# ALLabMTL/marl-demandresponse

Hardware: AMD Instinct MI355X
Metric: house-steps/s (env.step throughput) at 1M houses; % HBM roofline (higher is better)
Workload: dtype f64; 1 GPU; 1,048,576 houses per GPU, random actions, fused FSM+thermal+reward step, every tick's reward row written (BASELINE metric at 1M houses; configs[1]'s controller); houses_per_gpu=1048576, houses_total=1048576, signal=sinusoidals, penalty=individual_L2, action_mode=random, chunk_ticks=128, window_ticks=32, parallelism=1 GPU

## Files before the change

### include/mdr.h

```cpp
#ifndef MDR_H_
#define MDR_H_

#include <stdint.h>

#ifdef __cplusplus
extern "C" {
#endif

#define MDR_ABI_VERSION 5
#define MDR_MAX_CAP 64

enum {
  MDR_OK = 0,
  MDR_EARG = -1,
  MDR_EHIP = -2,
  MDR_ERCCL = -3,
  MDR_ENOMEM = -4,
  MDR_ESTATE = -5,
};

enum { MDR_PEN_INDIVIDUAL_L2 = 0, MDR_PEN_COMMON_L2 = 1, MDR_PEN_COMMON_MAX = 2, MDR_PEN_MIXTURE = 3 };

enum {
  MDR_ACT_BUFFER = 0,
// ... 52 lines not shown
const char* mdr_build_id(void);
int mdr_abi_sizes(int64_t* out, int n);
const char* mdr_last_error(void);
int mdr_graph_info(mdr_ctx* ctx, int64_t* out, int n);
int mdr_graph_memset_probe(mdr_ctx* ctx, int64_t* out, int n, void* stream);
int mdr_create(mdr_ctx** out, const mdr_config* cfg);
int mdr_destroy(mdr_ctx* ctx);
int mdr_bind(mdr_ctx* ctx, const mdr_soa* soa);

int mdr_params_changed(mdr_ctx* ctx);

enum { MDR_OPT_STEP_TPW = 1, MDR_OPT_FASTDIV = 2, MDR_OPT_WINDOW_PIPELINE = 3, MDR_OPT_SHARDED_OVERLAP = 4,
       MDR_OPT_GREEDY_SORT = 5, MDR_OPT_FORCE_HALO = 6, MDR_OPT_WINDOW_THERMAL = 7,
       MDR_OPT_HALO_OVERLAP = 9, MDR_OPT_ACTOR_GENERIC = 10, MDR_OPT_HALO_IN_COUNTS = 12,
       MDR_OPT_GQ_BAND = 13, MDR_OPT_ACTOR_FP32_FORM = 14, MDR_OPT_GQ_FUSED = 15, MDR_OPT_GQ_ADAPTIVE = 16,
       MDR_OPT_ACTOR_GRID = 17 };
enum { MDR_FP32_F16_SPLIT = 0, MDR_FP32_BF16_SPLIT3 = 1 };
enum { MDR_THERMAL_EXACT = 0, MDR_THERMAL_AFFINE = 1 };
int mdr_set_option(mdr_ctx* ctx, int option, int64_t value);

size_t mdr_window_onb_bytes(int64_t n_local, int waves);
int mdr_window_geometry_check(int64_t n_local, size_t onb_bytes, size_t wah_bytes);
size_t mdr_window_pen_bytes(int64_t n_local);
int mdr_window_pen_check(int64_t n_local, size_t pen_bytes);
size_t mdr_window_stats_bytes(int64_t n_local);
int mdr_window_stats_check(int64_t n_local, size_t bytes);

typedef struct mdr_pop_spec {
  double target_temp, std_target;
  double thermo_lo, thermo_hi;
  double ca, cm, hm;
  double init_air, init_mass;
  int32_t n_draw;
  uint8_t draw_idx[MDR_MAX_CAP];
} mdr_pop_spec;
int mdr_populate(mdr_ctx* ctx, const mdr_pop_spec* spec, void* stream);

// ... 207 lines not shown
```

### marl-demandresponse_amd/csrc/mdr_capi.hip

```cpp
#include <hip/hip_ext.h>
#include <hip/hip_runtime.h>
#include <hipcub/hipcub.hpp>
#include <rccl/rccl.h>

#include <cmath>
#include <cstdio>
#include <cstdlib>
#include <cstring>
#include <map>
#include <string>
#include <tuple>
#include <vector>

#include "mdr_actor.h"
#include "mdr_devbuf.h"
#include "mdr_interp.h"
#include "mdr_obs_dev.h"
#include "mdr_kernels.h"

using namespace mdr;

namespace {

thread_local std::string g_err;
// ... 102 lines not shown
  bool actor_generic = false;
  int actor_grid = 0;
  bool actor_fp32_bf16 = false;
  bool halo_overlap = true;
  bool halo_in_counts = true;
  Dev<unsigned long long> d_c5;
  int thermal = MDR_THERMAL_AFFINE;
  int win = kWindowMax;
  Dev<unsigned long long> d_wslab;
  int wslab_len = 0;
  bool wslab_dirty = true;
  Dev<uint64_t> d_onb;
  Dev<uint32_t> d_wah;
  Dev<uint64_t> d_onb2;
  Dev<uint32_t> d_wah2;
  bool coef_dirty = true;
  Dev<int> d_flags;
  Dev<unsigned> d_tickets;
  Dev<TickArgs> d_ticks;
  std::map<GraphKey, std::pair<hipGraphExec_t, int>> graphs;
  int64_t g_cap = 0;
  Dev<double> g_key, g_key2, g_ps, g_incl;
  Dev<int> g_idx, g_idx2;
  Dev<uint8_t> g_ls;
  Dev<unsigned char> g_tmp;
  Dev<int64_t> g_kpos, g_extra;
  Dev<double> g_part;
  Dev<unsigned> g_hist;
  Dev<unsigned char> g_sel_rec;
  GqSel* g_sel = nullptr;
// ... 30 lines not shown
    void* user = nullptr;
  } host;
  int world = 1, rank = 0;
  hipStream_t comm_stream = nullptr;
  hipStream_t cap_stream = nullptr;
  hipEvent_t ev_k1[kSlabs] = {}, ev_ar[kSlabs] = {}, ev_pc = nullptr;
  hipEvent_t ev[16] = {};
  std::vector<hipEvent_t>* step_events = nullptr;
  struct {
    bool on = false;
    int n = 0, mode = 0;
    uint64_t tick0 = 0;
    const uint8_t* action = nullptr;
    int64_t act_stride = 0;
    bool sharded = false;
  } begun;
  Dev<unsigned char> d_actor;
  Dev<float> d_actor_raw;
  std::vector<int> actor_key;
  mdr_actor_spec actor{};
  mdr_actor_net net{};
  bool actor_ready = false;
  int actor_head = MDR_HEAD_SOFTMAX;
  Dev<float> d_eps;
  Dev<float> d_chain;
  int n_cu = 0;
  Dev<double> d_obs_sc;
  Dev<uint8_t> d_act;
  Dev<float> d_halo;
  Dev<double> d_stats;
// ... 342 lines not shown
    for (int i = 0; i < cfg->n_cap; ++i) ok = ok && fabs(tab[i]) < 1099511627776.0;
    k.fast_tick_ok = ok ? 1 : 0;
  }
  c->slab_len = kCountShards * cfg->n_cap;
  if (c->d_slab.reserve((size_t)kSlabs * c->slab_len))
    return cleanup(fail(MDR_ENOMEM, "count slabs"));
  if (hipMemset(c->d_slab, 0, kSlabs * c->slab_len * sizeof(unsigned long long)) != hipSuccess)
    return cleanup(fail(MDR_EHIP, "count slabs memset"));
  c->tpw = default_tpw(cfg->n_local);
  if (cfg->n_cap <= kWindowCap) {
    c->wslab_len = kWindowMax * kCountShards * cfg->n_cap + kWindowMax * cfg->n_cap + kWindowMax * kWindowRec;
    const size_t tiles64 = whole_blocks(win_tiles(cfg->n_local) + 1, kCountWaves) * kWinHpt + 1;
    if (c->d_wslab.reserve((size_t)3 * c->wslab_len) || c->d_onb.reserve(tiles64 * kWindowMax) ||
        c->d_wah.reserve((size_t)cfg->n_local + 1))
      return cleanup(fail(MDR_ENOMEM, "window count slabs"));
  } else {
    c->win = 0;
  }
  c->pen_blocks = (int)blocks(cfg->n_local, 512);
  if (c->d_pen_partial.reserve((size_t)2 * c->pen_blocks) || c->d_partial2.reserve(2))
    return cleanup(fail(MDR_ENOMEM, "penalty partials"));
  if (cfg->penalty_mode != MDR_PEN_INDIVIDUAL_L2 && c->d_wslab) {
    if (c->d_wpen.reserve(mdr_window_pen_bytes(cfg->n_local) / sizeof(double)) || c->d_wres.reserve(3 * kWindowMax))
      return cleanup(fail(MDR_ENOMEM, "window penalty partials"));
  }
  for (auto& e : c->ev)
    if (hipEventCreate(&e) != hipSuccess) return cleanup(fail(MDR_EHIP, "event"));
  for (int i = 0; i < kSlabs; ++i)
    if (hipEventCreateWithFlags(&c->ev_k1[i], hipEventDisableTiming) != hipSuccess ||
        hipEventCreateWithFlags(&c->ev_ar[i], hipEventDisableTiming) != hipSuccess)
// ... 66 lines not shown
    case MDR_OPT_ACTOR_GRID:
      if (value < 0) return fail(MDR_EARG, "mdr_set_option: ACTOR_GRID must be >= 0");
      c->actor_grid = (int)std::min<int64_t>(value, (int64_t)c->n_cu);
      break;
    case MDR_OPT_ACTOR_FP32_FORM:
      if (value != MDR_FP32_F16_SPLIT && value != MDR_FP32_BF16_SPLIT3)
        return fail(MDR_EARG, "mdr_set_option: ACTOR_FP32_FORM must be MDR_FP32_F16_SPLIT or MDR_FP32_BF16_SPLIT3");
      c->actor_fp32_bf16 = value == MDR_FP32_BF16_SPLIT3;
      c->actor_key.clear();
      break;
    case MDR_OPT_WINDOW_THERMAL:
      if (value != MDR_THERMAL_EXACT && value != MDR_THERMAL_AFFINE)
        return fail(MDR_EARG, "mdr_set_option: WINDOW_THERMAL must be MDR_THERMAL_EXACT or _AFFINE");
      c->thermal = (int)value;
      break;
    default: return fail(MDR_EARG, "mdr_set_option: unknown option");
  }
  HIP_TRY(hipDeviceSynchronize());
  destroy_graphs(c);
  return MDR_OK;
}

int mdr_bind(mdr_ctx* c, const mdr_soa* s) {
  drop_begun(c);
  if (!c || !s) return fail(MDR_EARG, "mdr_bind: null argument");
  if (!s->t_air || !s->t_mass || !s->hvac || !s->ua || !s->ca || !s->cm || !s->hm || !s->target ||
      !s->cap_idx)
    return fail(MDR_EARG, "mdr_bind: null array");
  KParams& k = c->kp;
  k.t_air = s->t_air;
// ... 171 lines not shown
}

static bool window_ok(const mdr_ctx* c, int mode) {
  return window_geom_ok(c) && (win_common(c) ? c->d_wpen != nullptr : true) &&
         (mode == MDR_ACT_RANDOM || mode == MDR_ACT_ALWAYS_ON || mode == MDR_ACT_BUFFER);
}

static bool closed_ok(const mdr_ctx* c, int mode, bool stats = false) {
  return window_geom_ok(c) && (win_common(c) ? !stats && c->d_wpen && c->d_wres : true) &&
         (mode == MDR_ACT_BANGBANG || mode == MDR_ACT_DEADBAND_BANGBANG);
}

static int wslab_clean(mdr_ctx* c, hipStream_t st) {
  if (!c->wslab_dirty || !c->d_wslab) return MDR_OK;
  HIP_TRY(hipMemsetAsync(c->d_wslab, 0, 3 * sizeof(unsigned long long) * c->wslab_len, st));
  c->wslab_dirty = false;
  return MDR_OK;
}

static unsigned win_grid(const mdr_ctx* c, int waves = 4) {
  return (unsigned)(whole_blocks(win_tiles(c->kp.n), waves) / waves);
}

extern "C" size_t mdr_window_onb_bytes(int64_t n_local, int waves) {
  if (n_local < 0 || waves < 1) return 0;
  return whole_blocks(win_tiles(n_local), waves) * kWinHpt * kWindowMax * sizeof(uint64_t);
}

extern "C" int mdr_window_geometry_check(int64_t n_local, size_t onb_bytes, size_t wah_bytes) {
  if (n_local < 1) return fail(MDR_EARG, "window launch: no houses");
  const size_t need = std::max(mdr_window_onb_bytes(n_local, kCountWaves), mdr_window_onb_bytes(n_local, 4));
  if (onb_bytes < need)
    return fail(MDR_EARG, "window launch: ON-mask rows of " + std::to_string(onb_bytes) + " B, the launch geometry touches " +
                              std::to_string(need) + " B");
  if (wah_bytes < (size_t)n_local * sizeof(uint32_t))
    return fail(MDR_EARG, "window launch: end-word buffer shorter than the shard");
  return MDR_OK;
}

extern "C" size_t mdr_window_pen_bytes(int64_t n_local) {
  if (n_local < 0) return 0;
  return whole_blocks(win_tiles(n_local), 4) * kWindowMax * 2 * sizeof(double);
}

extern "C" int mdr_window_pen_check(int64_t n_local, size_t pen_bytes) {
  if (n_local < 1) return fail(MDR_EARG, "window launch: no houses for the penalty partial rows");
  const size_t need = mdr_window_pen_bytes(n_local);
  if (pen_bytes < need)
    return fail(MDR_EARG, "window launch: penalty partial rows of " + std::to_string(pen_bytes) +
                              " B, the launch geometry writes " + std::to_string(need) + " B");
  return MDR_OK;
// ... 182 lines not shown
  for (int j = 0; j < K; ++j) {
    const mdr_tick& h = host_ticks[j];
    dv.od_k[j] = h.t_od_prev + 273.0;
    dv.solar[j] = h.solar;
    dv.s_prev[j] = h.s_prev;
    if (fabs(h.t_od_prev) < 1048576.0 && fabs(h.solar) < 1099511627776.0) dv.ok |= 1u << j;
  }
  dv.tick0 = host_ticks[0].tick;
  if (nw == 1) dv.p_out = a.p_out;
  if (first == kBegunAllreduced) dv.red = win_red_ptr(c, s.slot(0));
  if (int rc = s.step(0, nw > 1 ? s.plan.size(1) : 0, c->d_onb, c->d_wah, s.slot(1), &dv)) return rc;
  if (int rc = s.finish(0)) return rc;
  if (a.n > K)
    if (int rc = stage_recs(host_ticks + K, a.n - K, c->d_ticks + K, st)) return rc;
  if (int rc = s.staged_windows(1, false)) return rc;
  c->wslab_dirty = false;
  return MDR_OK;
}

static int window_pipeline(mdr_ctx* c, const RolloutArgs& a, hipStream_t st) {
  if (int rc = win_common_unsharded(c, true)) return rc;
  const WinSeq s{c, a, st, WinPlan(a.n, c->win)};
  const int nw = s.plan.count();
  hipStream_t cs = c->comm_stream;
  uint64_t* onbs[2] = {c->d_onb, c->d_onb2};
  uint32_t* wahs[2] = {c->d_wah, c->d_wah2};
  c->wslab_dirty = true;
  HIP_TRY(hipEventRecord(c->ev_pc, st));
  HIP_TRY(hipStreamWaitEvent(cs, c->ev_pc, 0));
  for (int w = 0; w < nw; ++w) {
// ... 267 lines not shown

int mdr_rollout_stats(mdr_ctx* c, int n, const mdr_tick* ticks, const uint8_t* action, int64_t act_stride,
                      int mode, double* reward, int64_t rew_stride, double* p_out, double* stats, int row0,
                      int use_graph, void* stream) {
  const RolloutArgs a{n, action, act_stride, mode, reward, rew_stride, p_out};
  const char* const who = stats ? "mdr_rollout_stats" : "mdr_rollout";
  if (int rc = rollout_preamble(c, who, ticks && a.reward, a, 0)) return rc;
  if (stats) {
    if (row0 < 0) return fail(MDR_EARG, std::string(who) + ": row0 < 0");
    if (int rc = rollout_stats_path(c, a.mode, who); rc < 0) return rc;
  }
  if (common_sharded(c))
    return fail(MDR_EARG, std::string(who) + ": common penalty modes on a sharded context need the per-step API");
  hipStream_t st = S(stream);
  double* const srow = stats ? stats + (size_t)row0 * kTickRow : nullptr;
  const bool counted = begun_matches(c, a, ticks, false);
  if (c->begun.on && !counted) c->wslab_dirty = true;
  c->begun.on = false;
  int rc = refresh_if_dirty(c, st);
  if (rc) return rc;
  if (counted || (!use_graph && window_ok(c, a.mode) && consecutive(ticks, a.n))) {
    rc = ensure_ticks(c, a.n);
    if (!rc) rc = wslab_clean(c, st);
    if (!rc) rc = window_launches_direct(c, a, ticks, counted ? kBegun : kCountNow, st);
    c->counts_ready = false;
    return rc;
  }
  rc = stage_ticks(c, a.n, ticks, st);
  if (!rc) rc = wslab_clean(c, st);
  if (!rc && stats) rc = rollout_stats_scratch(c, a.mode, !a.p_out);
  if (rc) return rc;
  if (!use_graph) {
    rc = rollout_launches(c, a, st, srow);
    c->counts_ready = false;
    return rc;
  }
  const GraphKey key{a, stats, stats ? row0 : 0};
  auto it = c->graphs.find(key);
  if (it == c->graphs.end()) {
// ... 22 lines not shown

int mdr_rollout_begin(mdr_ctx* c, int n, uint64_t tick0, const uint8_t* action, int64_t act_stride, int mode,
                      void* stream) {
  const RolloutArgs a{n, action, act_stride, mode, nullptr, 0, nullptr};
  if (int rc = rollout_preamble(c, "mdr_rollout_begin", true, a, 0)) return rc;
  if (c->begun.on) c->wslab_dirty = true;
  c->begun.on = false;
  if (!window_ok(c, mode)) return MDR_OK;
  const bool sharded = has_comm(c);
  if (sharded && n > c->win) return MDR_OK;
  if (common_sharded(c)) return MDR_OK;
  hipStream_t st = S(stream);
  int rc = refresh_if_dirty(c, st);
  if (!rc) rc = wslab_clean(c, st);
  if (rc) return rc;
  const int k0 = WinPlan(n, c->win).size(0);
  c->wslab_dirty = true;
  rc = launch_count(c, mode, action, act_stride, nullptr, tick0, k0, c->d_wslab, c->d_onb, c->d_wah, nullptr, st,
                    true);
  if (rc) return rc;
  if (sharded) {
    if (int rc2 = comm_allreduce(c, win_red_ptr(c, c->d_wslab), (size_t)k0 * c->kp.n_cap, 0, st)) return rc2;
  }
  c->wslab_dirty = false;
  c->begun = {true, n, mode, tick0, action, act_stride, sharded};
  return MDR_OK;
}

int mdr_time_step_kernels(mdr_ctx* c, int n, const mdr_tick* ticks, const uint8_t* action, int64_t act_stride,
                          int mode, double* reward, int64_t rew_stride, void* stream, float* ms, int* launches) {
// ... 1816 lines not shown
```

### marl-demandresponse_amd/csrc/mdr_kernels.h

```cpp
#pragma once
#include <hip/hip_runtime.h>
#include <stdint.h>

#include "../../include/mdr.h"

namespace mdr {

constexpr int kCountShards = 64;
constexpr int kWinShards = 16;
constexpr int kCountWaves = 16;
constexpr int kTicketGroups = 64;
constexpr int kTicketWords = 32 * (kTicketGroups + 1);
constexpr int kSlabs = 4;
constexpr int kObsBlock = 128;
constexpr int kActBangBang = 16;
constexpr int kActDeadband = 17;

struct KParams {
  int64_t n, goff, n_global;
  int dt, L, n_cap, penalty_mode;
  double deadband, alpha_temp, alpha_sig, norm_temp, norm_sig;
  double alpha_ind_l2, alpha_common_l2, alpha_common_max;
  uint64_t seed;
  double* t_air;
// ... 123 lines not shown
                              unsigned long long* slot, W... wstat);
__global__ void k_closed_reward(KParams p, const double* rec, int j0, double* reward, int64_t rew_stride);
__global__ void k_closed_reward_common(KParams p, const double* res, const double* rec, int j0, double* reward,
                                       int64_t rew_stride);
__global__ void k_win_shard_sum(KParams p, unsigned long long* slot);
__global__ void k_closed_reward_sharded(KParams p, const unsigned long long* red, const TickArgs* tkp, int j0, int nt,
                                        double* reward, int64_t rew_stride, double* p_out);
__global__ void k_reward_finalize_dev(KParams p, const TickArgs* tkp, const unsigned long long* counts,
                                      const double* partial2, double* reward);
__global__ void k_win_reduce(KParams p, unsigned long long* slot, int nt, const TickArgs* tkp, double* p_out);
__global__ void k_win_records(KParams p, unsigned long long* slot, int nt, const TickArgs* tkp, double* p_out);
template <int ACT, int HPT>
__global__ void k_count_window(KParams p, const uint8_t* action, int64_t act_stride, const TickArgs* tkp,
                               uint64_t tick0, int nt, unsigned long long* slot, uint64_t* onb, uint32_t* wah,
                               const uint32_t* w_in, unsigned* ticket);
__global__ void k_probe_stream(KParams p, double* reward);
__global__ void k_refresh(KParams p, int* params_bad);
__global__ void k_div_check(const double* a, const double* b, int64_t n, unsigned long long* mismatches);
__global__ void k_pen_reduce(const double* pen_partial, int nblk, double* partial2);
__global__ void k_reward_finalize(KParams p, TickArgs tk, const unsigned long long* counts,
                                  const double* partial2, double* reward);
__global__ void k_reward_state(KParams p, const TickArgs* tkp, const unsigned long long* counts,
                               double* reward, double* p_out);
__global__ void k_populate(KParams p, PopArgs a);
constexpr int kStats = 12;
constexpr int kStatsBlocks = 512;
__global__ void k_cluster_stats(KParams p, const double* reward, double* partial);
__global__ void k_cluster_stats_final(const double* partial, int nblk, double* out);
constexpr int kTickRow = 16;
constexpr int kTickBlock = 256;
// ... 101 lines not shown
```

### marl-demandresponse_amd/csrc/mdr_kernels.hip

```cpp
#include "mdr_kernels.h"

#include <tuple>
#include <type_traits>

#include "mdr_device.h"
#include "mdr_obs_dev.h"

namespace mdr {


__device__ __forceinline__ void count_on(bool on, int cls, int n_cap, unsigned* hist,
                                         unsigned long long* slab) {
  const int lane = threadIdx.x & 63;
  for (int k = 0; k < n_cap; ++k) {
    const unsigned long long m = __ballot(on && cls == k);
    if (lane == 0 && m) atomicAdd(&hist[k], (unsigned)__popcll(m));
  }
  __syncthreads();
  if ((int)threadIdx.x < n_cap) {
    const unsigned v = hist[threadIdx.x];
    if (v) atomicAdd(&slab[(blockIdx.x % kCountShards) * n_cap + threadIdx.x],
                     (unsigned long long)v);
  }
}
// ... 933 lines not shown
    if (__hip_atomic_fetch_add(&tickets[32 * g], 1u, __ATOMIC_RELAXED, __HIP_MEMORY_SCOPE_AGENT) == gsize - 1u) {
      __hip_atomic_store(&tickets[32 * g], 0u, __ATOMIC_RELAXED, __HIP_MEMORY_SCOPE_AGENT);
      unsigned* top = &tickets[32 * kTicketGroups];
      if (__hip_atomic_fetch_add(top, 1u, __ATOMIC_RELAXED, __HIP_MEMORY_SCOPE_AGENT) == G - 1u) {
        __hip_atomic_store(top, 0u, __ATOMIC_RELAXED, __HIP_MEMORY_SCOPE_AGENT);
        last = 1u;
      }
    }
    s_last = last;
  }
  __syncthreads();
  return s_last != 0u;
}

template <int NTH>
__device__ void win_reduce_last(const KParams& p, unsigned long long* __restrict__ slot, int nt,
                                unsigned* __restrict__ ticket) {
  static_assert(kWinShards == 16, "one 16-lane group per entry");
  constexpr int EPT = kWinMax * kWinCap * kWinShards / NTH;
  constexpr int EPK = NTH / 16;
  __shared__ unsigned long long s_red[kWinMax * kWinCap];
  if (!grid_last_block(ticket)) return;
  __builtin_amdgcn_fence(__ATOMIC_ACQUIRE, "wavefront");
  const int ncap = p.n_cap, E = nt * ncap, sh = threadIdx.x & 15;
  unsigned long long v[EPT];
#pragma unroll
  for (int k = 0; k < EPT; ++k) {
    const int e = (int)(threadIdx.x >> 4) + EPK * k;
    v[k] = 0ull;
    if (e < E) {
      const int j = e / ncap, c = e - j * ncap;
      v[k] = __hip_atomic_load(&slot[((size_t)j * kCountShards + sh) * ncap + c], __ATOMIC_RELAXED,
                               __HIP_MEMORY_SCOPE_AGENT);
    }
  }
#pragma unroll
  for (int k = 0; k < EPT; ++k) {
    const int e = (int)(threadIdx.x >> 4) + EPK * k;
// ... 3 lines not shown
                         __HIP_MEMORY_SCOPE_AGENT);
    }
    unsigned long long x = v[k];
#pragma unroll
    for (int off = 8; off > 0; off >>= 1) x += __shfl_xor(x, off);
    if (sh == 0 && e < E) s_red[e] = x;
  }
  __syncthreads();
  for (int e = threadIdx.x; e < E; e += blockDim.x) win_red(slot, ncap)[e] = s_red[e];
  if ((int)threadIdx.x < nt) {
    double p_on[kWinCap];
#pragma unroll
    for (int k = 0; k < kWinCap; ++k) p_on[k] = p.p_on[k < ncap ? k : 0];
    win_rec(slot, ncap)[threadIdx.x * kWinRec] = win_power(p, s_red + threadIdx.x * ncap, p_on);
  }
}

template <int HPT>
struct WinTile {
  uint32_t tile, i0;
  uint32_t idx[HPT];
  bool v[HPT];
  uint64_t g0;
  int sh;
  __device__ __forceinline__ WinTile(const KParams& p) {
    const uint32_t n = (uint32_t)p.n;
    const uint32_t wv = (uint32_t)__builtin_amdgcn_readfirstlane((int)(threadIdx.x >> 6));
    tile = blockIdx.x * (blockDim.x >> 6) + wv;
    i0 = tile * (64u * HPT) + (uint32_t)(threadIdx.x & 63);
#pragma unroll
// ... 137 lines not shown
#pragma unroll
  for (int h = 0; h < HPT; ++h) {
    w[h] = w_in ? w_in[t.idx[h]] : p.hvac[t.idx[h]];
    cls[h] = p.cap_idx[t.idx[h]];
  }
  uint64_t cm[HPT][kWinCap];
  win_classes<HPT>(t, cls, cm);
  win_run<ACT, HPT>(p, w, cm, t, tkp, tick0, nt, action, act_stride, s_cnt[wv],
                    onb + (size_t)t.tile * HPT * kWinMax);
#pragma unroll
  for (int h = 0; h < HPT; ++h)
    if (t.v[h]) wah[t.i0 + 64u * h] = w[h];
  __syncthreads();
  win_flush<kCountWaves>(p, nt, s_cnt, slot);
  if (ticket) win_reduce_last<64 * kCountWaves>(p, slot, nt, ticket);
}

struct AffWin {
  double tt, tm, tq, to, qt;
  double mt, mm, mq, mo, qm;
};

__device__ __forceinline__ AffWin aff_window(double ua, double ca, double cm, double hm, double dt, double qc,
                                             bool fast) {
  const RcCoef k = fast ? rc_coeffs_t<true>(ua, ca, cm, hm, dt) : rc_coeffs_t<false>(ua, ca, cm, hm, dt);
  const double iD = 1.0 / (k.r2 - k.r1), iCa = 1.0 / ca, iUa = 1.0 / ua;
  const double a_t = (k.r2 + (ua + hm) * iCa) * iD;
  const double a_m = -(hm * iCa) * iD;
  const double a_q = -(iCa + k.r2 * iUa) * iD;
  const double a_o = -(ua * iCa + k.r2) * iD;
// ... 228 lines not shown

  if (la_K > 0) {
    uint64_t cmk[HPT][kWinCap];
    win_classes<HPT>(t, cls, cmk);
    win_run<ACT, HPT>(p, w_end, cmk, t, KA ? nullptr : tkp + K, KA ? dv.tick0 + (uint64_t)K : 0, la_K,
                      ACT == MDR_ACT_BUFFER ? action + (int64_t)K * act_stride : nullptr, act_stride, s_cnt[wv],
                      onb_w);
#pragma unroll
    for (int h = 0; h < HPT; ++h)
      if (t.v[h]) wah[t.i0 + 64u * h] = w_end[h];
    __syncthreads();
    win_flush(p, la_K, s_cnt, next_slot);
  }
}

constexpr int kClosedSums = 8;
constexpr int kClosedTr = 68;
struct ClosedLds {
  double tr[4][kClosedSums + 1][kClosedTr];
  double ws[4][kWinMax][kStats];
};
__device__ __forceinline__ ClosedLds& closed_lds() {
  __shared__ ClosedLds s;
  return s;
}
template <bool STATS> struct ClosedAcc {};
template <> struct ClosedAcc<true> {
  double a[kClosedSums], mx;
  uint32_t n_lock, n_on;
};
// ... 261 lines not shown
                                                                      unsigned long long*, WinDrv, WinPen);
#define MDR_INST_WIN_F(A, SI, KA_, FO) MDR_INST_WIN_C(A, SI, KA_, FO, false)
#define MDR_INST_WIN(A)                                                                                         \
  MDR_INST_WIN_C(A, false, false, MDR_THERMAL_EXACT, true) MDR_INST_WIN_C(A, false, true, MDR_THERMAL_EXACT, true)   \
  MDR_INST_WIN_C(A, false, false, MDR_THERMAL_AFFINE, true) MDR_INST_WIN_C(A, false, true, MDR_THERMAL_AFFINE, true) \
  MDR_INST_WIN_F(A, true, false, MDR_THERMAL_EXACT) MDR_INST_WIN_F(A, false, false, MDR_THERMAL_EXACT)          \
  MDR_INST_WIN_F(A, true, true, MDR_THERMAL_EXACT) MDR_INST_WIN_F(A, false, true, MDR_THERMAL_EXACT)            \
  MDR_INST_WIN_F(A, true, false, MDR_THERMAL_AFFINE) MDR_INST_WIN_F(A, false, false, MDR_THERMAL_AFFINE)        \
  MDR_INST_WIN_F(A, true, true, MDR_THERMAL_AFFINE) MDR_INST_WIN_F(A, false, true, MDR_THERMAL_AFFINE)          \
  template __global__ void k_count_window<A, kWinHpt>(KParams, const uint8_t*, int64_t, const TickArgs*, uint64_t, \
                                                      int, unsigned long long*, uint64_t*, uint32_t*, const uint32_t*, \
                                                      unsigned*);
MDR_INST_WIN(MDR_ACT_RANDOM)
MDR_INST_WIN(MDR_ACT_ALWAYS_ON)
MDR_INST_WIN(MDR_ACT_BUFFER)

#define MDR_INST_PIPE(T, A, LA, G)                                                                    \
  template __global__ void k_step_pipe<T, A, LA, G>(KParams, const uint8_t*, TickArgs, const TickArgs*, \
                                                    const unsigned long long*, double*, double*,         \
                                                    unsigned long long*, unsigned long long*, GqOut, GqfBufs, int);
MDR_INST_PIPE(1, MDR_ACT_RANDOM, MDR_ACT_RANDOM, 0)
MDR_INST_PIPE(2, MDR_ACT_RANDOM, MDR_ACT_RANDOM, 0)
MDR_INST_PIPE(4, MDR_ACT_RANDOM, MDR_ACT_RANDOM, 0)
MDR_INST_PIPE(8, MDR_ACT_RANDOM, MDR_ACT_RANDOM, 0)
MDR_INST_PIPE(2, MDR_ACT_BUFFER, 0, 0)
MDR_INST_PIPE(4, MDR_ACT_BUFFER, 0, 0)
MDR_INST_PIPE(2, MDR_ACT_BUFFER, 0, 1)
MDR_INST_PIPE(4, MDR_ACT_BUFFER, 0, 1)
MDR_INST_PIPE(2, MDR_ACT_BUFFER, 0, 2)
MDR_INST_PIPE(4, MDR_ACT_BUFFER, 0, 2)
// ... 2310 lines not shown
```

### marl-demandresponse_amd/mdr_amd/_lib.py

```python
from __future__ import annotations

import ctypes as C
import os
import threading

HERE = os.path.dirname(os.path.abspath(__file__))
LIB_PATH = os.environ.get("MDR_LIB", os.path.join(HERE, "libmdr_hip.so"))

ABI_VERSION = 5
MAX_CAP = 64

ACT_BUFFER, ACT_RANDOM, ACT_ALWAYS_ON, ACT_BANGBANG, ACT_DEADBAND_BANGBANG = 0, 1, 2, 16, 17
CTRL_NONE, CTRL_BANGBANG, CTRL_DEADBAND_BANGBANG, CTRL_GREEDY_KEYS = 0, 1, 2, 3
COMM_RING, COMM_TABLE = 0, 1
PEN_MODES = {"individual_L2": 0, "common_L2": 1, "common_max_error": 2, "mixture": 3}
ERRORS = {-1: "MDR_EARG", -2: "MDR_EHIP", -3: "MDR_ERCCL", -4: "MDR_ENOMEM", -5: "MDR_ESTATE"}
OPTIONS = {"step_tpw": 1, "fastdiv": 2, "window_pipeline": 3, "sharded_overlap": 4, "greedy_sort": 5, "halo_overlap": 9, "actor_generic": 10,
           "force_halo": 6, "window_thermal": 7, "halo_in_counts": 12,
           "gq_band": 13, "actor_fp32_form": 14, "gq_fused": 15, "gq_adaptive": 16, "actor_grid": 17}
THERMAL_EXACT, THERMAL_AFFINE = 0, 1
FP32_F16_SPLIT, FP32_BF16_SPLIT3 = 0, 1
HEADS = {"softmax": 0, "q": 1}


class MdrLibraryError(RuntimeError):
    """libmdr_hip.so is missing or unusable (no CPU fallback exists)."""


class MdrError(RuntimeError):
    pass


class mdr_config(C.Structure):
    _fields_ = [
# ... 89 lines not shown
    "mdr_last_error": (C.c_char_p, []),
    "mdr_graph_info": (I, [VP, P(I64), I]),
    "mdr_graph_memset_probe": (I, [VP, P(I64), I, VP]),
    "mdr_actor_status": (I, [VP, P(I64), I, VP]),
    "mdr_actor_set_head": (I, [VP, I, C.c_float, VP]),
    "mdr_greedy_fused_diag": (I, [VP, P(U64)]),
    "mdr_greedy_fused_stamps": (I, [VP, I, P(U64)]),
    "mdr_create": (I, [P(VP), P(mdr_config)]),
    "mdr_destroy": (I, [VP]),
    "mdr_bind": (I, [VP, P(mdr_soa)]),
    "mdr_params_changed": (I, [VP]),
    "mdr_set_rollout_window": (I, [VP, I]),
    "mdr_set_option": (I, [VP, I, I64]),
    "mdr_window_onb_bytes": (C.c_size_t, [I64, I]),
    "mdr_window_geometry_check": (I, [I64, C.c_size_t, C.c_size_t]),
    "mdr_window_pen_bytes": (C.c_size_t, [I64]),
    "mdr_window_pen_check": (I, [I64, C.c_size_t]),
    "mdr_window_stats_bytes": (C.c_size_t, [I64]),
    "mdr_window_stats_check": (I, [I64, C.c_size_t]),
    "mdr_time_step_kernels": (I, [VP, I, VP, VP, I64, I, VP, I64, VP, P(C.c_float), P(I)]),
    "mdr_rollout_begin": (I, [VP, I, U64, VP, I64, I, VP]),
    "mdr_populate": (I, [VP, P(mdr_pop_spec), VP]),
    "mdr_power_counts": (I, [VP, VP, I, U64, VP]),
    "mdr_counts_buffer": (I, [VP, P(VP), P(I)]),
    "mdr_step": (I, [VP, VP, I, P(mdr_tick), VP, I, I, VP, VP, VP]),
    "mdr_penalty_partials": (I, [VP, VP]),
    "mdr_penalty_buffer": (I, [VP, P(VP)]),
    "mdr_reward_finalize": (I, [VP, P(mdr_tick), VP, VP]),
    "mdr_rollout": (I, [VP, I, VP, VP, I64, I, VP, I64, VP, I, VP]),
    "mdr_rollout_stats": (I, [VP, I, VP, VP, I64, I, VP, I64, VP, VP, I, I, VP]),
# ... 168 lines not shown
```

Baseline: 414.8 billion house-steps/s.

## Group four rollout windows per count and step kernel launch

Adds a windowed rollout path, on by default, that batches up to four consecutive tick windows into one count kernel and one step kernel. House state (temperatures, thermal coefficients, HVAC words) stays in registers across the grouped windows instead of being reloaded and stored for each window, and fewer kernels are launched. It uses extra count slabs and ON-mask buffers and a separate records kernel per group. Each group still needs count, records and step launches in sequence, and the larger per-group working set could affect cache behaviour.

New measurement: 407.8 billion house-steps/s (median of 2 runs). No clear change (-1.7%).

```diff
diff --git a/include/mdr.h b/include/mdr.h
--- a/include/mdr.h
+++ b/include/mdr.h
@@ -90,13 +90,15 @@
        MDR_OPT_GREEDY_SORT = 5, MDR_OPT_FORCE_HALO = 6, MDR_OPT_WINDOW_THERMAL = 7,
        MDR_OPT_HALO_OVERLAP = 9, MDR_OPT_ACTOR_GENERIC = 10, MDR_OPT_HALO_IN_COUNTS = 12,
        MDR_OPT_GQ_BAND = 13, MDR_OPT_ACTOR_FP32_FORM = 14, MDR_OPT_GQ_FUSED = 15, MDR_OPT_GQ_ADAPTIVE = 16,
-       MDR_OPT_ACTOR_GRID = 17 };
+       MDR_OPT_ACTOR_GRID = 17, MDR_OPT_WINDOW_CALL = 18 };
 enum { MDR_FP32_F16_SPLIT = 0, MDR_FP32_BF16_SPLIT3 = 1 };
 enum { MDR_THERMAL_EXACT = 0, MDR_THERMAL_AFFINE = 1 };
 int mdr_set_option(mdr_ctx* ctx, int option, int64_t value);
 
 size_t mdr_window_onb_bytes(int64_t n_local, int waves);
 int mdr_window_geometry_check(int64_t n_local, size_t onb_bytes, size_t wah_bytes);
+size_t mdr_window_call_onb_bytes(int64_t n_local);
+int mdr_window_call_geometry_check(int64_t n_local, size_t onb_bytes, size_t wah_bytes, int slots);
 size_t mdr_window_pen_bytes(int64_t n_local);
 int mdr_window_pen_check(int64_t n_local, size_t pen_bytes);
 size_t mdr_window_stats_bytes(int64_t n_local);
diff --git a/marl-demandresponse_amd/csrc/mdr_capi.hip b/marl-demandresponse_amd/csrc/mdr_capi.hip
--- a/marl-demandresponse_amd/csrc/mdr_capi.hip
+++ b/marl-demandresponse_amd/csrc/mdr_capi.hip
@@ -140,6 +140,9 @@
   Dev<uint32_t> d_wah;
   Dev<uint64_t> d_onb2;
   Dev<uint32_t> d_wah2;
+  bool win_call = true;
+  Dev<unsigned long long> d_cslab;
+  Dev<uint64_t> d_conb;
   bool coef_dirty = true;
   Dev<int> d_flags;
   Dev<unsigned> d_tickets;
@@ -200,6 +203,7 @@
     const uint8_t* action = nullptr;
     int64_t act_stride = 0;
     bool sharded = false;
+    bool call = false;
   } begun;
   Dev<unsigned char> d_actor;
   Dev<float> d_actor_raw;
@@ -572,6 +576,9 @@
     if (c->d_wslab.reserve((size_t)3 * c->wslab_len) || c->d_onb.reserve(tiles64 * kWindowMax) ||
         c->d_wah.reserve((size_t)cfg->n_local + 1))
       return cleanup(fail(MDR_ENOMEM, "window count slabs"));
+    if (c->d_cslab.reserve((size_t)kCallWin * c->wslab_len) ||
+        c->d_conb.reserve(mdr_window_call_onb_bytes(cfg->n_local) / sizeof(uint64_t)))
+      return cleanup(fail(MDR_ENOMEM, "window group count slabs"));
   } else {
     c->win = 0;
   }
@@ -668,6 +675,7 @@
         return fail(MDR_EARG, "mdr_set_option: WINDOW_THERMAL must be MDR_THERMAL_EXACT or _AFFINE");
       c->thermal = (int)value;
       break;
+    case MDR_OPT_WINDOW_CALL: c->win_call = value != 0; break;
     default: return fail(MDR_EARG, "mdr_set_option: unknown option");
   }
   HIP_TRY(hipDeviceSynchronize());
@@ -869,6 +877,7 @@
 static int wslab_clean(mdr_ctx* c, hipStream_t st) {
   if (!c->wslab_dirty || !c->d_wslab) return MDR_OK;
   HIP_TRY(hipMemsetAsync(c->d_wslab, 0, 3 * sizeof(unsigned long long) * c->wslab_len, st));
+  if (c->d_cslab) HIP_TRY(hipMemsetAsync(c->d_cslab, 0, kCallWin * sizeof(unsigned long long) * c->wslab_len, st));
   c->wslab_dirty = false;
   return MDR_OK;
 }
@@ -890,6 +899,29 @@
                               std::to_string(need) + " B");
   if (wah_bytes < (size_t)n_local * sizeof(uint32_t))
     return fail(MDR_EARG, "window launch: end-word buffer shorter than the shard");
+  return MDR_OK;
+}
+
+static size_t call_onb_region_bytes(int64_t n_local) {
+  return std::max(mdr_window_onb_bytes(n_local, kCountWaves), mdr_window_onb_bytes(n_local, 4));
+}
+
+extern "C" size_t mdr_window_call_onb_bytes(int64_t n_local) {
+  if (n_local < 0) return 0;
+  return (size_t)kCallWin * call_onb_region_bytes(n_local);
+}
+
+extern "C" int mdr_window_call_geometry_check(int64_t n_local, size_t onb_bytes, size_t wah_bytes, int slots) {
+  if (n_local < 1) return fail(MDR_EARG, "window group launch: no houses");
+  const size_t need = mdr_window_call_onb_bytes(n_local);
+  if (onb_bytes < need)
+    return fail(MDR_EARG, "window group launch: ON-mask rows of " + std::to_string(onb_bytes) +
+                              " B, the launch geometry touches " + std::to_string(need) + " B");
+  if (wah_bytes < (size_t)n_local * sizeof(uint32_t))
+    return fail(MDR_EARG, "window group launch: end-word buffer shorter than the shard");
+  if (slots < kCallWin)
+    return fail(MDR_EARG, "window group launch: " + std::to_string(slots) + " count slots, a group uses " +
+                              std::to_string(kCallWin));
   return MDR_OK;
 }
 
@@ -1102,6 +1134,82 @@
   if (a.n > K)
     if (int rc = stage_recs(host_ticks + K, a.n - K, c->d_ticks + K, st)) return rc;
   if (int rc = s.staged_windows(1, false)) return rc;
+  c->wslab_dirty = false;
+  return MDR_OK;
+}
+
+static bool call_ok(const mdr_ctx* c, int n) {
+  return c->win_call && c->d_cslab && c->d_conb && !has_comm(c) && c->world == 1 && !win_common(c) &&
+         WinPlan(n, c->win).count() > 1;
+}
+
+static CallWin call_group(const WinPlan& plan, int w0) {
+  CallWin cw{};
+  cw.nw = std::min(kCallWin, plan.count() - w0);
+  for (int g = 0; g < cw.nw; ++g) {
+    cw.start[g] = plan.start(w0 + g) - plan.start(w0);
+    cw.size[g] = plan.size(w0 + g);
+  }
+  return cw;
+}
+
+static int call_geometry(const mdr_ctx* c) {
+  const int slots = c->wslab_len > 0 ? (int)(c->d_cslab.capacity() / (size_t)c->wslab_len) : 0;
+  return mdr_window_call_geometry_check(c->kp.n, dev_bytes(c->d_conb), dev_bytes(c->d_wah), slots);
+}
+
+static int launch_count_call(mdr_ctx* c, int mode, const uint8_t* action, int64_t act_stride, uint64_t tick0,
+                             const CallWin& cw, hipStream_t st) {
+  if (int rc = call_geometry(c)) return rc;
+  const unsigned grid = win_grid(c, kCountWaves);
+  const size_t region = call_onb_region_bytes(c->kp.n) / sizeof(uint64_t);
+#define MDR_COUNT(A)                                                                                           \
+  hipLaunchKernelGGL((k_count_call<A, kWinHpt>), dim3(grid), dim3(64 * kCountWaves), 0, st, c->kp, action, act_stride, \
+                     tick0, cw, c->d_cslab, (size_t)c->wslab_len, c->d_conb, region, c->d_wah, c->d_tickets)
+  if (mode == MDR_ACT_RANDOM) MDR_COUNT(MDR_ACT_RANDOM);
+  else if (mode == MDR_ACT_ALWAYS_ON) MDR_COUNT(MDR_ACT_ALWAYS_ON);
+  else MDR_COUNT(MDR_ACT_BUFFER);
+#undef MDR_COUNT
+  LAUNCH_CHECK("k_count_call");
+  return MDR_OK;
+}
+
+static int launch_step_call(mdr_ctx* c, const CallWin& cw, double* reward, int64_t rew_stride, hipStream_t st) {
+  if (int rc = call_geometry(c)) return rc;
+  const unsigned grid = win_grid(c);
+  const size_t region = call_onb_region_bytes(c->kp.n) / sizeof(uint64_t);
+#define MDR_SC(SI, FO)                                                                                         \
+  hipLaunchKernelGGL((k_step_call<kWinHpt, SI, FO>), dim3(grid), dim3(256), 0, st, c->kp, cw,                  \
+                     (const unsigned long long*)c->d_cslab, (size_t)c->wslab_len, reward, rew_stride,          \
+                     (const uint64_t*)c->d_conb, region, (const uint32_t*)c->d_wah)
+  const bool simple = win_simple(c);
+  if (c->thermal == MDR_THERMAL_AFFINE) {
+    if (simple) MDR_SC(true, MDR_THERMAL_AFFINE);
+    else MDR_SC(false, MDR_THERMAL_AFFINE);
+  } else {
+    if (simple) MDR_SC(true, MDR_THERMAL_EXACT);
+    else MDR_SC(false, MDR_THERMAL_EXACT);
+  }
+#undef MDR_SC
+  LAUNCH_CHECK("k_step_call");
+  return MDR_OK;
+}
+
+static int window_call_launches(mdr_ctx* c, const RolloutArgs& a, const mdr_tick* host_ticks, bool counted,
+                                hipStream_t st) {
+  const WinPlan plan(a.n, c->win);
+  c->wslab_dirty = true;
+  for (int w0 = 0; w0 < plan.count(); w0 += kCallWin) {
+    const CallWin cw = call_group(plan, w0);
+    const int t0 = plan.start(w0), nt = cw.start[cw.nw - 1] + cw.size[cw.nw - 1];
+    if (w0 > 0 || !counted)
+      if (int rc = launch_count_call(c, a.mode, a.act_row(t0), a.act_stride, host_ticks[t0].tick, cw, st)) return rc;
+    if (int rc = stage_recs(host_ticks + t0, nt, c->d_ticks + t0, st)) return rc;
+    hipLaunchKernelGGL(k_call_records, dim3(cw.nw), dim3(kWindowMax), 0, st, c->kp, c->d_cslab, (size_t)c->wslab_len,
+                       cw, (const TickArgs*)(c->d_ticks + t0), w0 + kCallWin >= plan.count() ? a.p_out : nullptr);
+    LAUNCH_CHECK("k_call_records");
+    if (int rc = launch_step_call(c, cw, a.rew_row(t0), a.rew_stride, st)) return rc;
+  }
   c->wslab_dirty = false;
   return MDR_OK;
 }
@@ -1399,15 +1507,19 @@
     return fail(MDR_EARG, std::string(who) + ": common penalty modes on a sharded context need the per-step API");
   hipStream_t st = S(stream);
   double* const srow = stats ? stats + (size_t)row0 * kTickRow : nullptr;
-  const bool counted = begun_matches(c, a, ticks, false);
+  const bool direct_ok = window_ok(c, a.mode) && consecutive(ticks, a.n);
+  const bool call = direct_ok && !stats && call_ok(c, a.n);
+  const bool counted = begun_matches(c, a, ticks, false) && c->begun.call == call;
   if (c->begun.on && !counted) c->wslab_dirty = true;
   c->begun.on = false;
   int rc = refresh_if_dirty(c, st);
   if (rc) return rc;
-  if (counted || (!use_graph && window_ok(c, a.mode) && consecutive(ticks, a.n))) {
+  if (counted || (!use_graph && direct_ok)) {
     rc = ensure_ticks(c, a.n);
     if (!rc) rc = wslab_clean(c, st);
-    if (!rc) rc = window_launches_direct(c, a, ticks, counted ? kBegun : kCountNow, st);
+    if (!rc)
+      rc = call ? window_call_launches(c, a, ticks, counted, st)
+                : window_launches_direct(c, a, ticks, counted ? kBegun : kCountNow, st);
     c->counts_ready = false;
     return rc;
   }
@@ -1460,6 +1572,13 @@
   int rc = refresh_if_dirty(c, st);
   if (!rc) rc = wslab_clean(c, st);
   if (rc) return rc;
+  if (call_ok(c, n)) {
+    c->wslab_dirty = true;
+    if (int rc2 = launch_count_call(c, mode, action, act_stride, tick0, call_group(WinPlan(n, c->win), 0), st)) return rc2;
+    c->wslab_dirty = false;
+    c->begun = {true, n, mode, tick0, action, act_stride, false, true};
+    return MDR_OK;
+  }
   const int k0 = WinPlan(n, c->win).size(0);
   c->wslab_dirty = true;
   rc = launch_count(c, mode, action, act_stride, nullptr, tick0, k0, c->d_wslab, c->d_onb, c->d_wah, nullptr, st,
diff --git a/marl-demandresponse_amd/csrc/mdr_kernels.h b/marl-demandresponse_amd/csrc/mdr_kernels.h
--- a/marl-demandresponse_amd/csrc/mdr_kernels.h
+++ b/marl-demandresponse_amd/csrc/mdr_kernels.h
@@ -161,6 +161,20 @@
 __global__ void k_count_window(KParams p, const uint8_t* action, int64_t act_stride, const TickArgs* tkp,
                                uint64_t tick0, int nt, unsigned long long* slot, uint64_t* onb, uint32_t* wah,
                                const uint32_t* w_in, unsigned* ticket);
+constexpr int kCallWin = 4;
+struct CallWin {
+  int nw;
+  int start[kCallWin], size[kCallWin];
+};
+template <int ACT, int HPT>
+__global__ void k_count_call(KParams p, const uint8_t* action, int64_t act_stride, uint64_t tick0, CallWin cw,
+                             unsigned long long* slot, size_t slot_len, uint64_t* onb, size_t onb_region,
+                             uint32_t* wah, unsigned* ticket);
+__global__ void k_call_records(KParams p, unsigned long long* slot, size_t slot_len, CallWin cw, const TickArgs* tkp,
+                               double* p_out);
+template <int HPT, bool SIMPLE, int FORM>
+__global__ void k_step_call(KParams p, CallWin cw, const unsigned long long* slot, size_t slot_len, double* reward,
+                            int64_t rew_stride, const uint64_t* onb, size_t onb_region, const uint32_t* wah);
 __global__ void k_probe_stream(KParams p, double* reward);
 __global__ void k_refresh(KParams p, int* params_bad);
 __global__ void k_div_check(const double* a, const double* b, int64_t n, unsigned long long* mismatches);
diff --git a/marl-demandresponse_amd/csrc/mdr_kernels.hip b/marl-demandresponse_amd/csrc/mdr_kernels.hip
--- a/marl-demandresponse_amd/csrc/mdr_kernels.hip
+++ b/marl-demandresponse_amd/csrc/mdr_kernels.hip
@@ -971,14 +971,11 @@
 }
 
 template <int NTH>
-__device__ void win_reduce_last(const KParams& p, unsigned long long* __restrict__ slot, int nt,
-                                unsigned* __restrict__ ticket) {
+__device__ __forceinline__ void win_reduce_slot(const KParams& p, unsigned long long* __restrict__ slot, int nt,
+                                                unsigned long long* s_red) {
   static_assert(kWinShards == 16, "one 16-lane group per entry");
   constexpr int EPT = kWinMax * kWinCap * kWinShards / NTH;
   constexpr int EPK = NTH / 16;
-  __shared__ unsigned long long s_red[kWinMax * kWinCap];
-  if (!grid_last_block(ticket)) return;
-  __builtin_amdgcn_fence(__ATOMIC_ACQUIRE, "wavefront");
   const int ncap = p.n_cap, E = nt * ncap, sh = threadIdx.x & 15;
   unsigned long long v[EPT];
 #pragma unroll
@@ -1012,6 +1009,15 @@
     for (int k = 0; k < kWinCap; ++k) p_on[k] = p.p_on[k < ncap ? k : 0];
     win_rec(slot, ncap)[threadIdx.x * kWinRec] = win_power(p, s_red + threadIdx.x * ncap, p_on);
   }
+}
+
+template <int NTH>
+__device__ void win_reduce_last(const KParams& p, unsigned long long* __restrict__ slot, int nt,
+                                unsigned* __restrict__ ticket) {
+  __shared__ unsigned long long s_red[kWinMax * kWinCap];
+  if (!grid_last_block(ticket)) return;
+  __builtin_amdgcn_fence(__ATOMIC_ACQUIRE, "wavefront");
+  win_reduce_slot<NTH>(p, slot, nt, s_red);
 }
 
 template <int HPT>
@@ -1179,6 +1185,58 @@
   __syncthreads();
   win_flush<kCountWaves>(p, nt, s_cnt, slot);
   if (ticket) win_reduce_last<64 * kCountWaves>(p, slot, nt, ticket);
+}
+
+template <int ACT, int HPT>
+__global__ void __launch_bounds__(64 * kCountWaves) k_count_call(KParams p, const uint8_t* __restrict__ action,
+                                                    int64_t act_stride, uint64_t tick0, CallWin cw,
+                                                    unsigned long long* __restrict__ slot, size_t slot_len,
+                                                    uint64_t* __restrict__ onb, size_t onb_region,
+                                                    uint32_t* __restrict__ wah, unsigned* __restrict__ ticket) {
+  __shared__ unsigned s_cnt[kCountWaves][kWinMax * kWinCap];
+  __shared__ unsigned long long s_red[kWinMax * kWinCap];
+  const int wv = threadIdx.x >> 6;
+  const WinTile<HPT> t(p);
+  uint32_t w[HPT];
+  int cls[HPT];
+#pragma unroll
+  for (int h = 0; h < HPT; ++h) {
+    w[h] = p.hvac[t.idx[h]];
+    cls[h] = p.cap_idx[t.idx[h]];
+  }
+  uint64_t cm[HPT][kWinCap];
+  win_classes<HPT>(t, cls, cm);
+  for (int g = 0; g < cw.nw; ++g) {
+    const int s0 = cw.start[g], nt = cw.size[g];
+    if (g) __syncthreads();
+    win_run<ACT, HPT>(p, w, cm, t, nullptr, tick0 + (uint64_t)s0, nt,
+                      ACT == MDR_ACT_BUFFER ? action + (int64_t)s0 * act_stride : nullptr, act_stride, s_cnt[wv],
+                      onb + (size_t)g * onb_region + (size_t)t.tile * HPT * kWinMax);
+    __syncthreads();
+    win_flush<kCountWaves>(p, nt, s_cnt, slot + (size_t)g * slot_len);
+  }
+#pragma unroll
+  for (int h = 0; h < HPT; ++h)
+    if (t.v[h]) wah[t.i0 + 64u * h] = w[h];
+  if (!grid_last_block(ticket)) return;
+  __builtin_amdgcn_fence(__ATOMIC_ACQUIRE, "wavefront");
+  for (int g = 0; g < cw.nw; ++g) {
+    if (g) __syncthreads();
+    win_reduce_slot<64 * kCountWaves>(p, slot + (size_t)g * slot_len, cw.size[g], s_red);
+  }
+}
+
+__global__ void __launch_bounds__(kWinMax) k_call_records(KParams p, unsigned long long* __restrict__ slot,
+                                                          size_t slot_len, CallWin cw,
+                                                          const TickArgs* __restrict__ tkp, double* p_out) {
+  const int g = blockIdx.x, j = threadIdx.x, ncap = p.n_cap;
+  if (g >= cw.nw || j >= cw.size[g]) return;
+  unsigned long long* s = slot + (size_t)g * slot_len;
+  double p_on[kWinCap];
+#pragma unroll
+  for (int k = 0; k < kWinCap; ++k) p_on[k] = p.p_on[k < ncap ? k : 0];
+  win_tick_record(p, win_red(s, ncap) + j * ncap, tkp[cw.start[g] + j], p_on, win_rec(s, ncap) + j * kWinRec,
+                  g == cw.nw - 1 && j == cw.size[g] - 1 ? p_out : nullptr);
 }
 
 struct AffWin {
@@ -1437,6 +1495,175 @@
   }
 }
 
+template <int HPT, bool SIMPLE, int FORM>
+__global__ void __launch_bounds__(256) k_step_call(KParams p, CallWin cw, const unsigned long long* __restrict__ slot,
+                                                   size_t slot_len, double* __restrict__ reward, int64_t rew_stride,
+                                                   const uint64_t* __restrict__ onb, size_t onb_region,
+                                                   const uint32_t* __restrict__ wah) {
+  constexpr bool AFF = FORM == MDR_THERMAL_AFFINE;
+  const WinTile<HPT> t(p);
+  const uint64_t* onb_t = onb + (size_t)t.tile * HPT * kWinMax;
+
+  double T[HPT], Tm[HPT], ua[HPT], hm[HPT], tg[HPT], ca[HPT], cm[HPT];
+  uint32_t w_end[HPT];
+  int cls[HPT];
+  const bool params_ok = !*p.params_bad && p.fast_tick_ok;
+#pragma unroll
+  for (int h = 0; h < HPT; ++h) {
+    const uint32_t i = t.idx[h];
+    T[h] = p.t_air[i]; Tm[h] = p.t_mass[i]; ua[h] = p.ua[i]; hm[h] = p.hm[i]; tg[h] = p.target[i];
+    ca[h] = p.ca[i]; cm[h] = p.cm[i];
+    w_end[h] = wah[i];
+    cls[h] = p.cap_idx[i];
+  }
+  double q_on[kWinCap];
+#pragma unroll
+  for (int c = 0; c < kWinCap; ++c) q_on[c] = p.q_on[c < p.n_cap ? c : 0];
+  double qc[HPT], lo_tg[HPT], hi_tg[HPT];
+#pragma unroll
+  for (int h = 0; h < HPT; ++h) {
+    qc[h] = q_on[0];
+#pragma unroll
+    for (int c = 1; c < kWinCap; ++c) qc[h] = cls[h] == c ? q_on[c] : qc[h];
+    hi_tg[h] = tg[h] + p.deadband / 2.0;
+    lo_tg[h] = tg[h] - p.deadband / 2.0;
+  }
+  RcWin rw[AFF ? 1 : HPT];
+  AffWin aw[AFF ? HPT : 1];
+  double tk[HPT], tmk[HPT], hk[HPT];
+  double csum[HPT];
+#pragma unroll
+  for (int h = 0; h < HPT; ++h) {
+    if constexpr (AFF) {
+      aw[h] = aff_window(ua[h], ca[h], cm[h], hm[h], (double)p.dt, qc[h], params_ok);
+      hk[h] = hi_tg[h] + 273.0;
+      const AffWin& a = aw[h];
+      csum[h] = a.tt + a.tm + a.tq + a.to + a.qt + a.mt + a.mm + a.mq + a.mo + a.qm;
+    } else if (params_ok) {
+      rw[h] = rc_window(ua[h], ca[h], cm[h], hm[h], (double)p.dt);
+    } else {
+      rw[h].k = rc_coeffs_t<false>(ua[h], ca[h], cm[h], hm[h], (double)p.dt);
+      rw[h].rCa.nb = -ca[h];
+      rw[h].rc.nb = -ua[h];
+      rw[h].rd.nb = -(rw[h].k.r2 - rw[h].k.r1);
+      rw[h].UaHm = ua[h] + hm[h];
+    }
+  }
+  const uint32_t rb = t.i0 * 8u;
+  const double nalpha = -p.alpha_temp;
+
+  for (int g = 0; g < cw.nw; ++g) {
+    const int K = cw.size[g];
+    const double* rec = reinterpret_cast<const double*>(win_red(const_cast<unsigned long long*>(slot) + (size_t)g * slot_len, p.n_cap) +
+                                                        (size_t)kWinMax * p.n_cap);
+    const uint64_t* onb_w = onb_t + (size_t)g * onb_region;
+    double* rew_g = reward + (int64_t)cw.start[g] * rew_stride;
+    bool win_finite = true;
+    if constexpr (AFF) {
+#pragma unroll
+      for (int h = 0; h < HPT; ++h) {
+        tk[h] = T[h] + 273.0;
+        tmk[h] = Tm[h] + 273.0;
+        const double s = csum[h] + tk[h] + tmk[h] + hk[h];
+        win_finite = win_finite && (s - s == 0.0);
+      }
+      win_finite = __all(win_finite);
+    }
+    double r_od = rec[0], r_sol = rec[1], r_sig = rec[2];
+    uint64_t r_ok = __double_as_longlong(rec[3]);
+    uint64_t r_on[HPT];
+#pragma unroll
+    for (int h = 0; h < HPT; ++h) r_on[h] = onb_w[h];
+    for (int j = 0; j < K; ++j) {
+      const double od_k = r_od, solar = r_sol, nsig = r_sig;
+      const bool tick_ok = r_ok != 0;
+      uint64_t on_m[HPT];
+#pragma unroll
+      for (int h = 0; h < HPT; ++h) on_m[h] = r_on[h];
+      const int jn = j + 1 < K ? j + 1 : j;
+      r_od = rec[jn * kWinRec + 0];
+      r_sol = rec[jn * kWinRec + 1];
+      r_sig = rec[jn * kWinRec + 2];
+      r_ok = __double_as_longlong(rec[jn * kWinRec + 3]);
+#pragma unroll
+      for (int h = 0; h < HPT; ++h) r_on[h] = onb_w[jn * HPT + h];
+      char* rrow = reinterpret_cast<char*>(rew_g + (int64_t)j * rew_stride);
+      auto reward_of = [&](int h, double Tn, double tkn, auto fast_c) {
+        constexpr bool F = decltype(fast_c)::value;
+        if (SIMPLE) {
+          if (AFF && F) {
+            const double x = tkn - hk[h];
+            return __builtin_fma(nalpha, x * x, nsig);
+          }
+          const double x = Tn - hi_tg[h];
+          const double pen = F ? x * x : deadband_l2_0(hi_tg[h], Tn);
+          return nalpha * pen + nsig;
+        }
+        double pen = 0.0;
+        if (hi_tg[h] < Tn) { const double x = Tn - hi_tg[h]; pen = x * x; }
+        else if (lo_tg[h] > Tn) { const double x = lo_tg[h] - Tn; pen = x * x; }
+        const double tpen = p.alpha_temp * pen;
+        return -((p.norm_temp == 1.0 ? tpen : tpen / p.norm_temp) + -nsig);
+      };
+      if constexpr (AFF) {
+        auto houses = [&](auto fast_c) {
+#pragma unroll
+          for (int h = 0; h < HPT; ++h) {
+            const AffWin& a = aw[h];
+            const bool on = __builtin_amdgcn_inverse_ballot_w64(on_m[h]);
+            const double ut = __builtin_fma(a.to, od_k, __builtin_fma(a.tq, solar, on ? a.qt : 0.0));
+            const double um = __builtin_fma(a.mo, od_k, __builtin_fma(a.mq, solar, on ? a.qm : 0.0));
+            const double tkn = __builtin_fma(a.tt, tk[h], __builtin_fma(a.tm, tmk[h], ut));
+            const double tmkn = __builtin_fma(a.mt, tk[h], __builtin_fma(a.mm, tmk[h], um));
+            tk[h] = tkn;
+            tmk[h] = tmkn;
+            const double r = reward_of(h, tkn - 273.0, tkn, fast_c);
+            if (t.v[h]) __builtin_nontemporal_store(r, reinterpret_cast<double*>(rrow + (rb + 512u * h)));
+          }
+        };
+        if (win_finite && tick_ok) houses(std::true_type());
+        else houses(std::false_type());
+      } else {
+        uint64_t ok_m = ~0ull;
+#pragma unroll
+        for (int h = 0; h < HPT; ++h)
+          ok_m &= __builtin_amdgcn_ballot_w64(fabs(T[h]) < 1048576.0) & __builtin_amdgcn_ballot_w64(fabs(Tm[h]) < 1048576.0);
+        const bool fast = params_ok && tick_ok && ok_m == __builtin_amdgcn_read_exec();
+        auto houses = [&](auto fast_c) {
+          constexpr bool F = decltype(fast_c)::value;
+#pragma unroll
+          for (int h = 0; h < HPT; ++h) {
+            const bool on = __builtin_amdgcn_inverse_ballot_w64(on_m[h]);
+            const double q = on ? qc[h] : 0.0;
+            double Tn, Tmn;
+            rc_apply_win<F>(T[h], Tm[h], ua[h], hm[h], rw[h], q, solar, od_k, Tn, Tmn);
+            T[h] = Tn;
+            Tm[h] = Tmn;
+            const double r = reward_of(h, Tn, 0.0, fast_c);
+            if (t.v[h]) __builtin_nontemporal_store(r, reinterpret_cast<double*>(rrow + (rb + 512u * h)));
+          }
+        };
+        if (fast) houses(std::true_type());
+        else houses(std::false_type());
+      }
+    }
+    if constexpr (AFF) {
+#pragma unroll
+      for (int h = 0; h < HPT; ++h) {
+        T[h] = tk[h] - 273.0;
+        Tm[h] = tmk[h] - 273.0;
+      }
+    }
+  }
+
+#pragma unroll
+  for (int h = 0; h < HPT; ++h)
+    if (t.v[h]) {
+      const uint32_t i = t.i0 + 64u * h;
+      p.t_air[i] = T[h]; p.t_mass[i] = Tm[h]; p.hvac[i] = w_end[h];
+    }
+}
+
 constexpr int kClosedSums = 8;
 constexpr int kClosedTr = 68;
 struct ClosedLds {
@@ -1728,6 +1955,21 @@
 MDR_INST_WIN(MDR_ACT_RANDOM)
 MDR_INST_WIN(MDR_ACT_ALWAYS_ON)
 MDR_INST_WIN(MDR_ACT_BUFFER)
+
+#define MDR_INST_COUNT_CALL(A)                                                                                   \
+  template __global__ void k_count_call<A, kWinHpt>(KParams, const uint8_t*, int64_t, uint64_t, CallWin,         \
+                                                    unsigned long long*, size_t, uint64_t*, size_t, uint32_t*,   \
+                                                    unsigned*);
+MDR_INST_COUNT_CALL(MDR_ACT_RANDOM)
+MDR_INST_COUNT_CALL(MDR_ACT_ALWAYS_ON)
+MDR_INST_COUNT_CALL(MDR_ACT_BUFFER)
+#define MDR_INST_STEP_CALL(SI, FO)                                                                               \
+  template __global__ void k_step_call<kWinHpt, SI, FO>(KParams, CallWin, const unsigned long long*, size_t,     \
+                                                        double*, int64_t, const uint64_t*, size_t, const uint32_t*);
+MDR_INST_STEP_CALL(true, MDR_THERMAL_EXACT)
+MDR_INST_STEP_CALL(false, MDR_THERMAL_EXACT)
+MDR_INST_STEP_CALL(true, MDR_THERMAL_AFFINE)
+MDR_INST_STEP_CALL(false, MDR_THERMAL_AFFINE)
 
 #define MDR_INST_PIPE(T, A, LA, G)                                                                    \
   template __global__ void k_step_pipe<T, A, LA, G>(KParams, const uint8_t*, TickArgs, const TickArgs*, \
diff --git a/marl-demandresponse_amd/mdr_amd/_lib.py b/marl-demandresponse_amd/mdr_amd/_lib.py
--- a/marl-demandresponse_amd/mdr_amd/_lib.py
+++ b/marl-demandresponse_amd/mdr_amd/_lib.py
@@ -17,7 +17,8 @@
 ERRORS = {-1: "MDR_EARG", -2: "MDR_EHIP", -3: "MDR_ERCCL", -4: "MDR_ENOMEM", -5: "MDR_ESTATE"}
 OPTIONS = {"step_tpw": 1, "fastdiv": 2, "window_pipeline": 3, "sharded_overlap": 4, "greedy_sort": 5, "halo_overlap": 9, "actor_generic": 10,
            "force_halo": 6, "window_thermal": 7, "halo_in_counts": 12,
-           "gq_band": 13, "actor_fp32_form": 14, "gq_fused": 15, "gq_adaptive": 16, "actor_grid": 17}
+           "gq_band": 13, "actor_fp32_form": 14, "gq_fused": 15, "gq_adaptive": 16, "actor_grid": 17,
+           "window_call": 18}
 THERMAL_EXACT, THERMAL_AFFINE = 0, 1
 FP32_F16_SPLIT, FP32_BF16_SPLIT3 = 0, 1
 HEADS = {"softmax": 0, "q": 1}
@@ -137,6 +138,8 @@
     "mdr_set_option": (I, [VP, I, I64]),
     "mdr_window_onb_bytes": (C.c_size_t, [I64, I]),
     "mdr_window_geometry_check": (I, [I64, C.c_size_t, C.c_size_t]),
+    "mdr_window_call_onb_bytes": (C.c_size_t, [I64]),
+    "mdr_window_call_geometry_check": (I, [I64, C.c_size_t, C.c_size_t, I]),
     "mdr_window_pen_bytes": (C.c_size_t, [I64]),
     "mdr_window_pen_check": (I, [I64, C.c_size_t]),
     "mdr_window_stats_bytes": (C.c_size_t, [I64]),
```
